# 2gunsu/monocon-pytorch

Measured on AMD Instinct MI355X. Metric: images/sec (384x1280) fwd+bwd, higher is better.
Workload: dtype f32 (f16x2); 1 GPU; train step B=32/GPU 3x384x1280 (configs[2] shape, fp32 values, mode f16x2); global_batch=32, parallelism=dp1, precision_mode=f16x2

## Files before the change

monocon-pytorch_amd/csrc/mc_internal.h:

```cpp
#pragma once
#include <hip/hip_runtime.h>

#include <cstdarg>
#include <cstdio>
#include <map>
#include <memory>
#include <string>
#include <tuple>
#include <unordered_map>
#include <vector>

#include "../../include/monocon_hip.h"
#include "conv_mfma.h"
#include "kernels.h"
#include "train.h"

using namespace mc;

struct TrainState;
struct CommState;

constexpr int MC_NUM_GRAD_BUCKETS = 4;
struct GradBucket {
    float *p = nullptr;
// ... 8 lines not shown
int mc_comm_join(mc_handle *h, hipStream_t main);

struct Bound {
    void *ptr;
    int64_t numel;
    int dtype;
};

struct Tensor {
    float *p = nullptr;
    int B = 0, H = 0, W = 0, C = 0;
    unsigned *amax = nullptr;
    const float *la = nullptr, *lb = nullptr;
    bool lrelu = true;
    size_t numel() const { return (size_t)B * H * W * C; }
};
inline Tensor operand_tensor(const float *p, int B, int H, int W, int C) {
    Tensor t;
    t.p = const_cast<float *>(p); t.B = B; t.H = H; t.W = W; t.C = C;
    return t;
}

struct ConvLayer {
    std::string conv, bn;
    int ks = 1, stride = 1, cin = 0, cout = 0, coutp = 0, cfg = 0;
    float bn_eps = 1e-5f;
    float *wpk = nullptr, *scale = nullptr, *shift = nullptr;
    void *wpk16 = nullptr;
    unsigned *w_amax = nullptr;
};

inline bool conv_fwd_args(ConvPlan &p, const ConvLayer &L, const std::vector<const Tensor *> &srcs, int prec) {
    ConvArgs &a = p.a;
    const Tensor &s0 = *srcs[0];
    a.nsrc = (int)srcs.size();
    a.Cin = 0;
    for (int i = 0; i < a.nsrc; ++i) {
        a.src[i] = ConvSrc{srcs[i]->p, srcs[i]->C, srcs[i]->la, srcs[i]->lb};
        a.Cin += srcs[i]->C;
    }
    a.B = s0.B; a.Hin = s0.H; a.Win = s0.W;
    a.Hout = conv_out_dim(s0.H, L.ks, L.stride); a.Wout = conv_out_dim(s0.W, L.ks, L.stride);
    a.Cout = L.cout; a.CoutP = L.coutp; a.wpk = L.wpk;
    a.wpk16 = L.wpk16; a.prec = L.wpk16 ? prec : 0;
    if (a.prec == 3) {
        for (int i = 0; i < a.nsrc; ++i) a.amax_in[i] = srcs[i]->amax;
        a.amax_w = L.w_amax;
    }
    p.ks = L.ks; p.stride = L.stride;
    conv_plan(p);
    return a.Cin == L.cin;
}
inline void wgrad_args(WgradPlan &p, const std::vector<const Tensor *> &srcs, const Tensor &dy, int dy_ld, int Cout, int ks,
                       int stride, int prec) {
    WgradArgs &a = p.a;
    const Tensor &s0 = *srcs[0];
    a.nsrc = (int)srcs.size();
    a.Cin = 0;
    for (int i = 0; i < a.nsrc; ++i) {
        a.src[i] = ConvSrc{srcs[i]->p, srcs[i]->C, srcs[i]->la, srcs[i]->lb};
        a.amax_x[i] = srcs[i]->amax;
        a.Cin += srcs[i]->C;
    }
    a.amax_dy = dy.amax;
    a.B = s0.B; a.Hin = s0.H; a.Win = s0.W; a.Hout = dy.H; a.Wout = dy.W; a.Cout = Cout;
    a.dy = dy.p; a.dy_ld = dy_ld;
    a.prec = prec; p.ks = ks; p.stride = stride;
    wgrad_plan(p);
}

struct DeconvLayer {
    std::string name;
    int C = 0;
    float *wpk = nullptr;
};

constexpr const char *HEAD_NAMES[NUM_HEADS] = {"heatmap_head", "wh_head", "offset_head", "center2kpt_offset_head",
                                               "kpt_heatmap_head", "kpt_heatmap_offset_head", "dim_head", "depth_head",
                                               "dir_feat"};
struct HeadOutLayer { std::string layer; int row0, rows; };
struct HeadKeys { std::string conv3, attn; std::vector<HeadOutLayer> out; };
inline HeadKeys mc_head_keys(int hd) {
    const std::string pre = std::string("head.") + HEAD_NAMES[hd];
    const int r0 = head_row_begin()[hd], nr = head_row_begin()[hd + 1] - r0;
    HeadKeys k{pre + ".0", pre + ".1", {{pre + ".3", r0, nr}}};
    if (hd == NUM_HEADS - 1) k.out = {{"head.dir_cls.0", r0, nr / 2}, {"head.dir_reg.0", r0 + nr / 2, nr / 2}};
    return k;
}

enum StepKind { STEP_CONV, STEP_POOL, STEP_DECONV };
struct NetStep {
    StepKind kind;
    std::string name, bn;
    std::vector<int> srcs;
    int res = -1;
    int out = -1;
    int ks = 1, stride = 1, cout = 0;
    bool relu = true;
    bool dead = false;
    bool elementwise_consumers = false;
    bool never_lazy = false;
};
struct NetGraph {
    std::vector<NetStep> steps;
    std::vector<int> node_c;
    int lv[6] = {};
    int n_backbone = 0;
    int feat = -1;
};

struct PlanMem {
    std::vector<void *> bufs;
    size_t bytes = 0;
    unsigned *amax_arena = nullptr;
    int amax_used = 0;
    void release() {
        for (void *q : bufs) (void)hipFree(q);
        bufs.clear();
    }
};
// ... 146 lines not shown
```

monocon-pytorch_amd/csrc/mc_train_api.hip:

```cpp
#include "mc_internal.h"

#include <algorithm>
#include <cmath>
#include <cstdlib>
#include <cstring>
#include <vector>

static int check_targets(mc_handle *h, const mc_targets *t, const char *who) {
    if (!t) return fail(h, "%s: targets is NULL", who);
    const void *p[] = {t->center_heatmap_target, t->wh_target, t->offset_target, t->dim_target, t->alpha_cls_target,
                       t->alpha_offset_target, t->depth_target, t->center2kpt_offset_target, t->kpt_heatmap_target,
                       t->kpt_heatmap_offset_target, t->indices, t->indices_kpt, t->mask_target,
                       t->mask_center2kpt_offset, t->mask_kpt_heatmap_offset};
    for (size_t i = 0; i < sizeof(p) / sizeof(p[0]); ++i)
        if (!p[i]) return fail(h, "%s: targets field %d is NULL", who, (int)i);
    return 0;
}

extern "C" {

int mc_make_targets(mc_handle *h, const mc_labels *lab, int B, int max_objs, int pad_h, int pad_w, int fh, int fw,
                    const mc_targets *t, void *stream) {
    if (!h) return -1;
    if (!lab || !lab->gt_bboxes || !lab->gt_labels || !lab->gt_bboxes_3d || !lab->depths || !lab->gt_kpts_2d ||
// ... 107 lines not shown
    HIPCHK(h, mc::launch_focal(preds[0], t->center_heatmap_target, (size_t)B * 3 * HW, h->loss_ws, scratch_losses + 0, aux + 0, st));
    HIPCHK(h, mc::launch_focal(preds[1], t->kpt_heatmap_target, (size_t)B * 9 * HW, h->loss_ws + npf, scratch_losses + 5, aux + 1, st));
    if (h->dp_arena && dpreds[2] == h->dp_arena) {
        HIPCHK(h, hipMemsetAsync(h->dp_arena, 0, h->dp_arena_bytes, st));
    } else {
        for (int i = 2; i < 10; ++i) HIPCHK(h, hipMemsetAsync(dpreds[i], 0, (size_t)B * mc::PRED_CH[i] * HW * 4, st));
    }
    HIPCHK(h, mc::launch_focal_grad(preds[0], t->center_heatmap_target, (size_t)B * 3 * HW, aux + 0, grad_losses, 0, dpreds[0], st, wrt_pred));
    HIPCHK(h, mc::launch_focal_grad(preds[1], t->kpt_heatmap_target, (size_t)B * 9 * HW, aux + 1, grad_losses, 5, dpreds[1], st, wrt_pred));
    mc::GatherLossArgs g{};
    fill_gather_args(g, preds, dpreds, t, B, max_objs, (int)HW, scratch_losses, aux + 2, grad_losses);
    g.wrt_pred = wrt_pred;
    g.partial = gather_ws(h);
    HIPCHK(h, mc::launch_gathered_losses(g, 1, st));
    return 0;
}

int mc_losses_backward(mc_handle *h, const float *const preds[MC_NUM_PREDS], const mc_targets *t, int B, int max_objs,
                       int fh, int fw, const float *grad_losses, float *const dpreds[MC_NUM_PREDS], void *stream) {
    return losses_backward_impl(h, preds, t, B, max_objs, fh, fw, grad_losses, dpreds, stream, 0);
}

int mc_losses_backward_pred(mc_handle *h, const float *const preds[MC_NUM_PREDS], const mc_targets *t, int B, int max_objs,
                            int fh, int fw, const float *grad_losses, float *const dpreds[MC_NUM_PREDS], void *stream) {
    return losses_backward_impl(h, preds, t, B, max_objs, fh, fw, grad_losses, dpreds, stream, 1);
}

int mc_op_conv_wgrad(mc_handle *h, const float *const src[], const int src_channels[], int nsrc, int B, int Hin, int Win,
                     const float *dy, int Cout, int ksize, int stride, float *dw_oihw, void *stream) {
    if (!h) return -1;
    if (!src || !src_channels || !dy || !dw_oihw || nsrc < 1 || nsrc > 4) return fail(h, "mc_op_conv_wgrad: bad argument");
    if (!((ksize == 3 && (stride == 1 || stride == 2)) || (ksize == 1 && stride == 1)))
        return fail(h, "mc_op_conv_wgrad: unsupported k=%d stride=%d", ksize, stride);
    if (Cout % 4) return fail(h, "mc_op_conv_wgrad: Cout must be a multiple of 4");
    HIPCHK(h, hipSetDevice(h->device));
    hipStream_t st = static_cast<hipStream_t>(stream);
    Tensor x[4];
    std::vector<const Tensor *> xs;
    for (int i = 0; i < nsrc; ++i) {
        if (!src[i] || src_channels[i] % 16) return fail(h, "mc_op_conv_wgrad: source %d needs C %% 16 == 0", i);
        x[i] = operand_tensor(src[i], B, Hin, Win, src_channels[i]);
        xs.push_back(&x[i]);
    }
    Tensor dyt = operand_tensor(dy, B, mc::conv_out_dim(Hin, ksize, stride), mc::conv_out_dim(Win, ksize, stride), Cout);
    ScratchBuf slots;
    if (h->prec == 3) {
        size_t n[4];
        for (int i = 0; i < nsrc; ++i) n[i] = x[i].numel();
        HIPCHK(h, op_amax_slots(slots, src, n, nsrc, dy, dyt.numel(), false, st));
        for (int i = 0; i < nsrc; ++i) x[i].amax = slots.as<unsigned>() + i * mc::AMAX_WORDS;
        dyt.amax = slots.as<unsigned>() + 4 * mc::AMAX_WORDS;
    }
    mc::WgradPlan p{};
    wgrad_args(p, xs, dyt, Cout, Cout, ksize, stride, h->prec);
    void *part = nullptr;
    HIPCHK(h, hipMalloc(&part, mc::wgrad_partial_floats(p) * sizeof(float)));
    p.a.partial = static_cast<float *>(part);
    hipError_t e = mc::launch_wgrad(p, dw_oihw, st);
    hipError_t e2 = hipStreamSynchronize(st);
    (void)hipFree(part);
    HIPCHK(h, e);
    HIPCHK(h, e2);
    return 0;
}

int mc_op_conv_dgrad(mc_handle *h, const float *dy, const float *weight_oihw, int B, int Hin, int Win, int CinTotal,
                     int c_off, int Cs, int Cout, int ksize, int stride, int accumulate, float *dx, void *stream) {
    if (!h) return -1;
    if (!dy || !weight_oihw || !dx) return fail(h, "mc_op_conv_dgrad: null argument");
    if (!((ksize == 3 && (stride == 1 || stride == 2)) || (ksize == 1 && stride == 1)))
        return fail(h, "mc_op_conv_dgrad: unsupported k=%d stride=%d", ksize, stride);
    if (Cout % 16 || Cs % 4 || c_off < 0 || c_off + Cs > CinTotal) return fail(h, "mc_op_conv_dgrad: bad channel arguments");
    if (stride == 2 && ((Hin | Win) & 1)) return fail(h, "mc_op_conv_dgrad: stride 2 needs even Hin, Win");
    HIPCHK(h, hipSetDevice(h->device));
    hipStream_t st = static_cast<hipStream_t>(stream);
    const int Ho = mc::conv_out_dim(Hin, ksize, stride), Wo = mc::conv_out_dim(Win, ksize, stride);
    const int nclass = stride == 2 ? 4 : 1;
    ScratchBuf slots;
    unsigned *dy_amax = nullptr, *w_amax = nullptr;
    if (h->prec == 3) {
        const size_t ndy = (size_t)B * Ho * Wo * Cout;
        HIPCHK(h, op_amax_slots(slots, &dy, &ndy, 1, weight_oihw, (size_t)Cout * CinTotal * ksize * ksize, true, st));
        dy_amax = slots.as<unsigned>();
        w_amax = dy_amax + 4 * mc::AMAX_WORDS;
    }
    ScratchBuf panel[4], panel16[4];
    mc::PackBatch pack;
    for (int c = 0; c < nclass; ++c) {
        const int cls = stride == 2 ? c : -1;
        const size_t pn = mc::dgrad_panel_elems(ksize, cls, Cout, Cs);
        HIPCHK(h, panel[c].alloc(pn * 4));
        HIPCHK(h, hipMemsetAsync(panel[c].p, 0, pn * 4, st));
        if (mc::panel_has_pieces(h->prec, Cout)) {
            const size_t bytes16 = pn * 2 * mc::split_pieces(h->prec);
            HIPCHK(h, panel16[c].alloc(bytes16));
            HIPCHK(h, hipMemsetAsync(panel16[c].p, 0, bytes16, st));
        }
        pack.add(mc::pack_job_dgrad(weight_oihw, Cout, CinTotal, ksize, c_off, Cs, Cout, cls, panel[c].as<float>(), panel16[c].p,
                                    h->prec, w_amax));
    }
    hipError_t e = pack.launch(st);
    for (int c = 0; c < nclass && e == hipSuccess; ++c) {
        mc::ConvPlan d;
        mc::dgrad_conv_args(d, pack.jobs[c], h->prec, dy, dy_amax, B, Ho, Wo, Cout, dx, Hin, Win, accumulate != 0);
        d.a.cfg = h->force_cfg;
        mc::conv_plan(d);
        e = mc::launch_conv(d, st);
// ... 165 lines not shown
```

monocon-pytorch_amd/csrc/mc_train_plan.hip:

```cpp
#include <atomic>
#include <deque>
#include <functional>

#include "mc_internal.h"

using namespace mc;

namespace {

using Fn = std::function<int(mc_handle *, hipStream_t)>;

struct PlanSwitches {
    long long lazy_z;
    long long lazy_min;
    long long lazy_feat;
    long long zbits;
    long long grad_pool;
    long long grad_pool_cool;
    long long head_dx_fuse;
    long long head_zskip;
    long long dgrad_s2_thin;
    long long stem_fuse;
    long long bm_epilogue;
    long long wres_bwd;
    long long dual_stream;
    int side_sync_lo = 0, side_sync_hi = 0;
    bool plan_debug = false;
};
const struct { const char *name; long long PlanSwitches::*field; long long def; } SWITCH_TABLE[] = {
    {"MONOCON_HIP_LAZY_Z", &PlanSwitches::lazy_z, 3},
    {"MONOCON_HIP_LAZY_MIN", &PlanSwitches::lazy_min, 900000},
    {"MONOCON_HIP_LAZY_FEAT", &PlanSwitches::lazy_feat, 0},
    {"MONOCON_HIP_ZBITS", &PlanSwitches::zbits, 1},
    {"MONOCON_HIP_GRAD_POOL", &PlanSwitches::grad_pool, 1},
    {"MONOCON_HIP_GRAD_POOL_COOL", &PlanSwitches::grad_pool_cool, 2},
    {"MONOCON_HIP_HEAD_DX_FUSE", &PlanSwitches::head_dx_fuse, 1},
    {"MONOCON_HIP_HEAD_ZSKIP", &PlanSwitches::head_zskip, 1},
    {"MONOCON_HIP_DGRAD_S2_THIN", &PlanSwitches::dgrad_s2_thin, 1},
    {"MONOCON_HIP_STEM_FUSE", &PlanSwitches::stem_fuse, 1},
    {"MONOCON_HIP_BM_EPILOGUE", &PlanSwitches::bm_epilogue, 1},
    {"MONOCON_HIP_WRES_BWD", &PlanSwitches::wres_bwd, 0},
    {"MONOCON_HIP_DUAL_STREAM", &PlanSwitches::dual_stream, 1},
};
PlanSwitches read_switches() {
    PlanSwitches sw{};
    std::string changed;
    for (const auto &d : SWITCH_TABLE) {
        const char *e = std::getenv(d.name);
        sw.*d.field = e ? std::atoll(e) : d.def;
        if (sw.*d.field != d.def) changed += std::string(" ") + d.name + "=" + std::to_string(sw.*d.field);
    }
    if (const char *e = std::getenv("MONOCON_HIP_SIDE_SYNC")) {
        if (std::sscanf(e, "%d:%d", &sw.side_sync_lo, &sw.side_sync_hi) != 2) sw.side_sync_lo = sw.side_sync_hi = 0;
        if (sw.side_sync_lo < sw.side_sync_hi) changed += std::string(" MONOCON_HIP_SIDE_SYNC=") + e;
    }
    sw.plan_debug = std::getenv("MONOCON_HIP_PLAN_DEBUG") != nullptr;
    if (sw.plan_debug && !changed.empty()) fprintf(stderr, "[plan] switches off their defaults:%s\n", changed.c_str());
    return sw;
}

struct PoolBwdArgs {
    const float *x, *dout, *la, *lb;
    float *dx, *stats;
    int B, H, W, C, acc;
};

struct LastWriter {
    enum Kind { NONE, DGRAD_CONV, POOL_BWD, DECONV_BWD } kind = NONE;
    union {
        ConvPlan *conv;
        PoolBwdArgs *pool;
        float **deconv_stats;
    };
    LastWriter() : conv(nullptr) {}
    LastWriter(ConvPlan *c) : kind(c ? DGRAD_CONV : NONE), conv(c) {}
    LastWriter(PoolBwdArgs *p) : kind(p ? POOL_BWD : NONE), pool(p) {}
    LastWriter(float **s) : kind(s ? DECONV_BWD : NONE), deconv_stats(s) {}
};

struct TNode {
    Tensor t;
    float *g = nullptr;
    bool ginit = false, needs_grad = true;
    LastWriter last;
};

enum RecKind { REC_STEM, REC_CONV, REC_POOL, REC_DECONV, REC_HEAD };
struct Rec {
    RecKind kind;
    ConvLayer *L = nullptr;
    DeconvLayer *D = nullptr;
    std::vector<int> srcs;
    int res = -1, z = -1, in = -1;
    bool relu = true, dead = false;
    Tensor y;
// ... 347 lines not shown
        float *dst = alloc(pn);
        void *dst16 = panel_has_pieces(h->prec, CoutPad) ? alloc((3 * pn + 1) / 2) : nullptr;
        ts->pack_batch.add(pack_job_dgrad(w, Cout, CinTotal, k, c_off, Cs, CoutPad, cls, dst, dst16, h->prec, w_slot(w)));
        return ts->pack_batch.jobs.back();
    }

    void emit_dgrad(const float *w_master, const Tensor &dy, int Cout_fwd, int CinTotal, int ks, int stride, int c_off, int srcnode,
                    int CoutPad) {
        TNode &sn = ts->nodes[srcnode];
        if (!sn.needs_grad) return;
        g_acquire(srcnode);
        auto dgrad_conv = [&](int cls, ConvPlan &d) {
            const PackJobDesc &p = pack_job(w_master, Cout_fwd, CinTotal, ks, c_off, sn.t.C, CoutPad, cls);
            dgrad_conv_args(d, p, h->prec, dy.p, dy.amax, dy.B, dy.H, dy.W, dy.C, sn.g, sn.t.H, sn.t.W, sn.ginit);
            d.a.cfg = ts->ok ? mc_choose_conv_cfg(h, d) : CFG_128x32;
        };
        if (stride == 2 && ks == 3) {
            if (2 * dy.H != sn.t.H || 2 * dy.W != sn.t.W) { ts->ok = false; h->err = "train plan: stride-2 dgrad shape mismatch"; }
            if (sw.dgrad_s2_thin && ts->ok && dgrad_s2_thin_ok(h->prec, ks, stride, dy.C, sn.t.C, CinTotal, c_off, dy.amax, w_slot(w_master), dy.H, dy.W)) {
                const float *dyp = dy.p;
                float *gp = sn.g;
                const int B = dy.B, Hd = dy.H, Wd = dy.W, Cd = dy.C, acc = sn.ginit ? 1 : 0;
                const unsigned *dmax = dy.amax, *wmax = w_slot(w_master);
                push_bwd([=](mc_handle *hh, hipStream_t st) {
                    HIPCHK(hh, launch_dgrad_s2_thin(dyp, B, Hd, Wd, Cd, w_master, CinTotal, c_off, gp, acc, dmax, wmax, st));
                    return 0;
                });
                wrote(srcnode);
                return;
            }
            for (int cls = 0; cls < 4; ++cls) {
                ConvPlan d;
                dgrad_conv(cls, d);
                conv_plan(d);
                push_bwd([=](mc_handle *hh, hipStream_t st) { HIPCHK(hh, launch_conv(d, st)); return 0; });
            }
            wrote(srcnode);
            return;
        }
        if (dy.H != sn.t.H || dy.W != sn.t.W) { ts->ok = false; h->err = "train plan: dgrad shape mismatch"; }
        ConvPlan d;
        dgrad_conv(-1, d);
        if (sw.wres_bwd < 2) d.a.cfg &= ~CFG_WRES;
        conv_plan(d);
        ts->dgrads.push_back(d);
        ConvPlan *dp = &ts->dgrads.back();
        push_bwd([=](mc_handle *hh, hipStream_t st) { HIPCHK(hh, launch_conv(*dp, st)); return 0; });
        wrote(srcnode, d.bm_ok ? dp : nullptr);
    }

    int emit_wgrad(const std::vector<int> &srcs, const Tensor &dy, int dy_ld, int Cout, int ks, int stride, float *dw) {
        WgradPlan p{};
        const std::vector<const Tensor *> xs = conv_sources(srcs);
        wgrad_args(p, xs, dy, dy_ld, Cout, ks, stride, h->prec);
        if (wgrad_any_lazy(p.a) && !wgrad_lazy_capable(p)) {
            for (int s_ : srcs) materialise(s_);
            wgrad_args(p, xs, dy, dy_ld, Cout, ks, stride, h->prec);
        }
        p.a.partial = alloc(wgrad_partial_floats(p));
        return push_bwd([=](mc_handle *hh, hipStream_t st) { HIPCHK(hh, launch_wgrad(p, dw, st)); return 0; }, ON_SIDE);
    }

    struct BnBwd { Tensor dy; float *coef; bool affine_skipped; };
    BnBwd bn_backward(const Rec &r, const std::string &bn, bool caller_forms_dy = false) {
        TNode &zn = ts->nodes[r.z];
        Tensor dy = r.y;
        dy.p = zn.g;
        dy.amax = slot();
        unsigned *dymax = dy.amax;
        const int B = r.y.B, C = r.y.C, rows = r.y.H * r.y.W;
        const float *yp = r.y.p, *gz = zn.g, *zp = zn.t.p, *gamma = P(bn + ".weight", C), *mean = r.mean, *rstd = r.rstd;
        float *dg = G(bn + ".weight", C), *db = G(bn + ".bias", C), *dyp = dy.p;
        float *coef = alloc((size_t)C * 4);
        const int relu = r.relu ? ((r.res < 0 && r.ca && r.cb) ? 2 : 1) : 0;
        const float *fa = r.ca, *fb = r.cb;
        float *gres = nullptr;
        int gmode = 0;
        if (r.res >= 0 && ts->nodes[r.res].needs_grad) {
            gres = g_acquire(r.res);
            gmode = ts->nodes[r.res].ginit ? 2 : 1;
            wrote(r.res);
        }
        const double n = (double)B * rows;
        auto step = [&](float *partial, int nbp, int cstride, bool reduce, bool affine) {
            double *fold = fold_scratch(nbp, C);
            const int arelu = reduce ? relu : 0;
            const float *aa = reduce ? fa : nullptr, *ab = reduce ? fb : nullptr;
            push_bwd([=](mc_handle *hh, hipStream_t st) {
                if (reduce) HIPCHK(hh, launch_chan_reduce(yp, gz, zp, nullptr, B, rows, C, 1, relu, partial, C, st, fa, fb));
                HIPCHK(hh, launch_bn_bwd_finalize(partial, nbp, cstride, n, C, gamma, mean, rstd, dg, db, coef, st, fold));
                if (affine)
                    HIPCHK(hh, launch_affine_bwd(gz, zp, yp, coef, B, (size_t)rows, C, 0, arelu, dyp, gres, gmode, st, aa, ab, nullptr,
                                                 nullptr, dymax));
                return 0;
            });
            return BnBwd{dy, coef, !affine};
        };
        const LastWriter last = zn.last;
        ConvPlan *lp = last.kind == LastWriter::DGRAD_CONV ? last.conv : nullptr;
        ConvArgs *lc = lp ? &lp->a : nullptr;
        if (sw.bm_epilogue == 0 || (sw.bm_epilogue > 1 && r.y.H * r.y.W > sw.bm_epilogue)) lc = nullptr;
        if (sw.plan_debug)
            fprintf(stderr, "[plan] bn_backward %-40s %4d ch %4dx%-4d relu %d res %d last-writer-conv %d\n", bn.c_str(), C, r.y.H,
                    r.y.W, relu, r.res >= 0, lc != nullptr);
        if (lc && lc->out == zn.g && lc->Cout == C && lc->out_ld == C && lc->Hout == r.y.H && lc->Wout == r.y.W && !lc->stats) {
            const int ppi = lp->stat_rows, nbp = B * ppi, cstride = lc->CoutP;
            float *partial = alloc((size_t)nbp * cstride * 2);
            lc->stats = partial;
            lc->bm_y = yp; lc->bm_z = zp; lc->bm_a = fa; lc->bm_b = fb; lc->bm_relu = relu;
            lc->bm_zbits = relu == 1 ? r.zbits : nullptr;
// ... 617 lines not shown
```

monocon-pytorch_amd/csrc/train.h:

```cpp
#pragma once
#include <hip/hip_runtime.h>
#include <stdint.h>
#include <cstdlib>
#include <vector>

#include "conv_mfma.h"

namespace mc {

struct TargetArgs {
    const float *gt_bboxes, *gt_labels, *gt_bboxes_3d, *depths, *gt_kpts_2d, *gt_kpts_valid, *mask;
    int B, max_objs, num_kpt, num_classes, fh, fw;
    float h_ratio, w_ratio;
    float *center_heatmap, *kpt_heatmap;
    float *wh, *offset, *dim, *alpha_cls, *alpha_offset, *depth, *c2k, *kho;
    long long *indices, *indices_kpt;
    uint8_t *mask_target;
    float *mask_c2k, *mask_kho;
};
hipError_t launch_make_targets(const TargetArgs &a, hipStream_t st);

hipError_t launch_focal(const float *p, const float *t, size_t n, float *partial, float *loss_out, float *aux,
                        hipStream_t st);
hipError_t launch_focal_grad(const float *p, const float *t, size_t n, const float *aux, const float *gscale, int gidx,
// ... 141 lines not shown
int affine_bwd_blocks(int B, size_t rows_per_img, int C);
size_t colsum_partial_floats(size_t rows, int ld);
hipError_t launch_colsum(const float *x, size_t rows, int C, int ld, float *partial, float *out, hipStream_t st);
hipError_t launch_colsum_final(const float *partial, int nb, int C, float *out, hipStream_t st);
hipError_t launch_maxpool2_bwd(const float *x, const float *dout, int B, int H, int W, int C, float *dx, int accumulate,
                               hipStream_t st, const float *la = nullptr, const float *lb = nullptr,
                               float *stats_partial = nullptr);
int maxpool2_bwd_blocks(int B, int H, int W, int C);
size_t deconv4_bwd_w_partial_floats(int B, int H, int C);
hipError_t launch_deconv4_bwd_w(const float *in, const float *dout, int B, int H, int W, int C, float *partial, float *dw,
                                hipStream_t st, const float *la, const float *lb,
                                const float *wpk, float *din,
                                float *stats = nullptr);

hipError_t launch_dpred_pack(const float *const dpred[10], int ld, int B, int HW, float *out, hipStream_t st,
                             unsigned *nz = nullptr);
hipError_t launch_dpred_pack_user(const float *const dpred[10], const float *const pred[10], const float *const grad[10], int ld,
                                  int B, int HW, float *out, hipStream_t st, unsigned *nz = nullptr);
struct AttnTrainArgs {
    const float *stats;
    int chunks, stat_ld, B, HW;
    double *stats64;
    float *rm[9], *rv[9];
    long long *nbt[9];
    const float *att_w[9], *att_g[9], *att_b[9];
    float *att_rm[9], *att_rv[9];
    long long *att_nbt[9];
    const float *weight_[9], *bias_[9];
    float *sv_inst;
    float *mu_r;
    float *bn10;
    float *that, *yatt;
    float *gamma_p;
    float *scale, *shift;
};
struct AttnGradPtrs { float *d_weight_[9], *d_bias_[9], *d_att_w[9], *d_att_g[9], *d_att_b[9]; };
hipError_t launch_attn_train_fwd(const AttnTrainArgs &a, hipStream_t st);
hipError_t launch_attn_train_bwd(const AttnTrainArgs &a, const float *partial, int rb_per_img, const AttnGradPtrs &gp,
                                 float *coef, hipStream_t st);
hipError_t launch_head_bwd(const float *draw, int ld, const float *z, const float *x, const float *w1, int B, int HW,
                           int blocks, float *d, float *dw_partial, float *red_partial, hipStream_t st,
                           const float *scale = nullptr, const float *shift = nullptr, const unsigned *nz = nullptr);
hipError_t launch_head_dx(const float *draw, int ld, const float *x, const float *w1, const float *coef, int B, int HW, int blocks,
                          float *dx, float *csum, float *csum_out, unsigned *amax, hipStream_t st, const float *scale,
                          const float *shift, const unsigned *nz = nullptr);
hipError_t launch_splitk_reduce(const float *partial, int ksplit, int T, int Cout, int Cin, float *dw, hipStream_t st);
int stem_wgrad_blocks(int B, int H, int W);
hipError_t launch_stem_wgrad(const float *img, const float *dy, int B, int H, int W, float *partial, float *dw,
                             hipStream_t st, const unsigned *img_amax = nullptr, const unsigned *dy_amax = nullptr,
                             const float *y = nullptr, const float *coef = nullptr, const unsigned *y_amax = nullptr);
hipError_t launch_stem_dgrad(const float *dy, const float *w_oihw, int B, int H, int W, float *dx, hipStream_t st,
                             const float *y = nullptr, const float *coef = nullptr);

enum WgKernel { WG_FP32, WG_SPLIT, WG_PIPE, WG_SMALL, WG_THIN16 };
struct WgradArgs {
    ConvSrc src[4];
    int nsrc;
    int B, Hin, Win, Hout, Wout, Cin, Cout;
    const float *dy;
    int dy_ld;
    float *partial;
    int ksplit, n_tiles, c_tiles, ppr, ppi, groups_per_img;
    int kernel;
    int prec;
    int pb;
    int pipe;
    const unsigned *amax_x[4], *amax_dy;
};
static_assert(sizeof(WgradArgs) == 264, "WgradArgs is the kernels' parameter block: keep its layout");
struct WgradPlan {
    WgradArgs a;
    int ks, stride;
    int WN, WC;
    bool lazy_ok;
    bool ok;
    size_t partial_floats;
};
inline void wgrad_set_patches(WgradArgs &a, int pb) {
    a.ppr = (a.Wout + 7) / 8;
    a.ppi = a.ppr * ((a.Hout + 3) / 4);
    a.groups_per_img = (a.ppi + pb - 1) / pb;
}
inline bool wgrad_any_lazy(const WgradArgs &a) { return any_lazy_src(a.src, a.nsrc); }
template <int WN_, int WC_>
struct WgTile { static constexpr int WN = WN_, WC = WC_; };
template <typename F>
inline hipError_t with_wgrad_tile(int WN, int WC, F &&f) {
    if (WN == 2 && WC == 2) return f(WgTile<2, 2>{});
    if (WN == 4) return f(WgTile<4, 1>{});
    if (WN == 2) return f(WgTile<2, 1>{});
    return f(WgTile<1, 1>{});
}
inline size_t wgrad_lds_request(size_t need) {
#ifdef MC_DEBUG_HOOKS
    static const size_t pad = [] { const char *e = std::getenv("MONOCON_HIP_WGRAD_LDS_KB"); return e ? (size_t)std::atoi(e) * 1024 : (size_t)0; }();
    return pad > need ? pad : need;
#else
    return need;
#endif
}
void wgrad_plan(WgradPlan &p);
hipError_t launch_wgrad(const WgradPlan &p, float *dw_oihw, hipStream_t st);
inline size_t wgrad_partial_floats(const WgradPlan &p) { return p.partial_floats; }
inline bool wgrad_lazy_capable(const WgradPlan &p) { return p.lazy_ok; }
bool wgrad_is_small(const WgradArgs &a, int ks, int stride);
bool wgrad_thin_ok(const WgradArgs &a, int ks, int stride);
int wgrad_pipe_tile(const WgradArgs &a, int ks, int stride);
void wgrad_shape(const WgradArgs &a, int *WN, int *WC);
bool wgrad_sources_ok(const WgradArgs &a);
bool wgrad_bf16_ok(const WgradArgs &a, int ks, int stride);
hipError_t launch_wgrad_fp32(const WgradPlan &p, hipStream_t st);
hipError_t launch_wgrad_small(const WgradPlan &p, hipStream_t st);
hipError_t launch_wgrad_bf16(const WgradPlan &p, hipStream_t st);
hipError_t launch_wgrad_pipe(const WgradPlan &p, hipStream_t st);
hipError_t launch_wgrad_thin(const WgradPlan &p, hipStream_t st);

}
```

monocon-pytorch_amd/csrc/wgrad_plan.hip:

```cpp
#include <algorithm>
#include <cstdlib>
#include "conv_mfma.h"
#include "train.h"

namespace mc {

static int env_int(const char *name, int unset) { const char *e = std::getenv(name); return e ? std::atoi(e) : unset; }

void wgrad_plan(WgradPlan &p) {
    WgradArgs &a = p.a;
    const int ks = p.ks, stride = p.stride;
    a.pipe = p.WN = p.WC = 0; p.ok = true;
    if (wgrad_is_small(a, ks, stride)) {
        a.kernel = wgrad_thin_ok(a, ks, stride) ? WG_THIN16 : WG_SMALL;
        p.lazy_ok = a.prec == 3 && (a.kernel == WG_THIN16 || (stride == 2 && a.Cout == 32));
        const int rows = a.B * a.Hout;
        a.ksplit = std::min(rows / 4 > 0 ? rows / 4 : 1, 1024);
        a.n_tiles = a.c_tiles = 1; a.ppr = a.ppi = a.groups_per_img = 0;
    } else {
        int budget, WK = 1;
        if (const int tile = wgrad_pipe_tile(a, ks, stride)) {
            a.kernel = WG_PIPE; a.pipe = tile; a.pb = 1;
            p.WN = tile == 1 ? 4 : 2; p.WC = tile == 2 ? 4 : 2; WK = tile == 3 ? 2 : 1;
            p.lazy_ok = tile == 4;
            budget = env_int("MONOCON_HIP_WGRAD_PIPE_BLOCKS", 256);
        } else {
            wgrad_shape(a, &p.WN, &p.WC);
            const bool b16 = a.prec >= 1 && wgrad_bf16_ok(a, ks, stride), src_ok = wgrad_sources_ok(a);
            a.kernel = b16 ? WG_SPLIT : WG_FP32;
            a.pb = (b16 && a.prec >= 2) ? 1 : 2;
            p.lazy_ok = a.prec == 3 && b16 && src_ok;
            p.ok = src_ok && (b16 || (ks == 3 && (stride == 1 || stride == 2)) || (ks == 1 && stride == 1));
            budget = env_int("MONOCON_HIP_WGRAD_BLOCKS", 512) * 4 / (p.WN * p.WC);
        }
        a.n_tiles = (a.Cout + 32 * p.WN - 1) / (32 * p.WN);
        a.c_tiles = (a.Cin + 32 * p.WC - 1) / (32 * p.WC);
        wgrad_set_patches(a, a.pb);
        const long long G = (long long)a.B * a.groups_per_img;
        a.ksplit = (int)std::min<long long>(std::max(budget / (a.n_tiles * a.c_tiles), 1), G) * WK;
    }
    if (wgrad_any_lazy(a) && !p.lazy_ok) p.ok = false;
    p.partial_floats = (size_t)a.ksplit * ks * ks * a.Cout * a.Cin;
}

hipError_t launch_wgrad(const WgradPlan &p, float *dw_oihw, hipStream_t st) {
    const WgradArgs &a = p.a;
    if (!p.ok) return hipErrorInvalidValue;
    prof_last = {2, 2.0 * a.B * a.Hout * a.Wout * (double)a.Cout * a.Cin * p.ks * p.ks,
                 4.0 * ((double)a.B * a.Hin * a.Win * a.Cin + (double)a.B * a.Hout * a.Wout * a.Cout + (double)p.ks * p.ks * a.Cin * a.Cout)};
    hipError_t e = hipErrorInvalidValue;
    switch (a.kernel) {
    case WG_FP32: e = launch_wgrad_fp32(p, st); break;
    case WG_SPLIT: e = launch_wgrad_bf16(p, st); break;
    case WG_PIPE: e = launch_wgrad_pipe(p, st); break;
    case WG_SMALL: e = launch_wgrad_small(p, st); break;
    case WG_THIN16: e = launch_wgrad_thin(p, st); break;
    }
    if (e != hipSuccess) return e;
    return launch_splitk_reduce(a.partial, a.ksplit, p.ks * p.ks, a.Cout, a.Cin, dw_oihw, st);
}

}
```

scratch/wgrad_plan_dump.hip:

```cpp
#include <cstdio>
#include <cstdlib>
#include <cstring>
#include <string>
#include <vector>
#include "train.h"

using namespace mc;

struct Case { std::string name; int B, H, W; std::vector<int> cins; int Cout, ks, stride, dy_ld = 0; bool amax = true; };

static unsigned g_slot[4];
static bool g_probe = false, g_kernels = false;

static void fill(WgradArgs &a, const Case &c, int prec, int lazy) {
    a.nsrc = (int)c.cins.size();
    a.Cin = 0;
    const float *f = reinterpret_cast<const float *>(g_slot);
    for (int i = 0; i < a.nsrc; ++i) {
        const bool lz = lazy == 1 || (lazy == 2 && i == 0);
        a.src[i] = ConvSrc{f, c.cins[i], lz ? f : nullptr, lz ? f : nullptr};
        a.amax_x[i] = (prec == 3 && c.amax) ? g_slot : nullptr;
        a.Cin += c.cins[i];
    }
    a.amax_dy = (prec == 3 && c.amax) ? g_slot : nullptr;
    a.B = c.B; a.Hin = c.H; a.Win = c.W;
    a.Hout = conv_out_dim(c.H, c.ks, c.stride); a.Wout = conv_out_dim(c.W, c.ks, c.stride);
    a.Cout = c.Cout; a.dy = f; a.dy_ld = c.dy_ld ? c.dy_ld : c.Cout;
    a.prec = prec;
}

static void dump(const Case &c, int prec, int lazy) {
    size_t partial;
    bool lazy_ok;
    int small, pipe, bf16;
    hipError_t e = hipSuccess;
    char extra[64] = "";
#ifdef WGRAD_DUMP_OLD_API
    WgradArgs a{};
    fill(a, c, prec, lazy);
    wgrad_plan(a, c.ks, c.stride);
    partial = wgrad_partial_floats(a, c.ks);
    lazy_ok = wgrad_lazy_capable(a, c.ks, c.stride);
    small = a.small; pipe = a.pipe;
    bf16 = !a.small && !a.pipe && a.prec >= 1 && wgrad_bf16_ok(a, c.ks, c.stride);
    if (g_probe) e = launch_wgrad(a, c.ks, c.stride, nullptr, 0);
#else
    WgradPlan p{};
    fill(p.a, c, prec, lazy);
    p.ks = c.ks; p.stride = c.stride;
    wgrad_plan(p);
    const WgradArgs &a = p.a;
    partial = wgrad_partial_floats(p);
    lazy_ok = wgrad_lazy_capable(p);
    small = a.kernel == WG_SMALL || a.kernel == WG_THIN16; pipe = a.pipe; bf16 = a.kernel == WG_SPLIT;
    if (g_probe) e = launch_wgrad(p, nullptr, 0);
    static const char *const names[] = {"fp32", "split", "pipe", "small", "thin16"};
    if (g_kernels) std::snprintf(extra, sizeof extra, " kernel=%s waves=%dx%d", names[a.kernel], p.WN, p.WC);
#endif
    std::printf("%s prec=%d lazy=%d ksplit=%d n_tiles=%d c_tiles=%d pb=%d ppr=%d ppi=%d groups_per_img=%d partial=%zu lazy_ok=%d "
                "small=%d pipe=%d bf16=%d launch=%s%s\n",
                c.name.c_str(), prec, lazy, a.ksplit, a.n_tiles, a.c_tiles, a.pb, a.ppr, a.ppi, a.groups_per_img, partial, (int)lazy_ok,
                small, pipe, bf16, !g_probe ? "-" : (e == hipErrorInvalidValue ? "invalid" : "ok"), extra);
}

static void train_plan_cases(std::vector<Case> &out, int B, int H, int W) {
    char tag[32];
    std::snprintf(tag, sizeof tag, "plan_b%d_%dx%d", B, H, W);
    auto add = [&](const char *what, int level, std::vector<int> cins, int Cout, int ks, int stride, int dy_ld = 0) {
        out.push_back({std::string(tag) + "_" + what, B, H >> level, W >> level, std::move(cins), Cout, ks, stride, dy_ld});
    };
    add("level0", 0, {16}, 16, 3, 1);
    add("level1", 0, {16}, 32, 3, 2);
    const int ch[6] = {16, 32, 64, 128, 256, 512};
    for (int lv = 2; lv <= 5; ++lv) {
        const int ci = ch[lv - 1], co = ch[lv];
        const std::string l = "level" + std::to_string(lv);
        add((l + "_down").c_str(), lv - 1, {ci}, co, 3, 2);
        add((l + "_block").c_str(), lv, {co}, co, 3, 1);
        add((l + "_project").c_str(), lv, {ci}, co, 1, 1);
        add((l + "_root").c_str(), lv, lv == 5 ? std::vector<int>{co, co, ci} : std::vector<int>{co, co}, co, 1, 1);
        if (lv == 3 || lv == 4) add((l + "_root4").c_str(), lv, {co, co, ci, co}, co, 1, 1);
    }
    for (int lv = 5; lv >= 3; --lv) {
        const int co = ch[lv - 1];
        add(("ida_proj_" + std::to_string(ch[lv]) + "_" + std::to_string(co)).c_str(), lv, {ch[lv]}, co, 3, 1);
        add(("ida_node_" + std::to_string(co)).c_str(), lv - 1, {co, co}, co, 3, 1);
    }
    add("heads_64_576", 2, {64}, 576, 3, 1, 576);
}

static void test_cases(std::vector<Case> &out) {
    out.insert(out.end(), {
        {"wg_s1_64_64", 2, 16, 24, {64}, 64, 3, 1}, {"wg_s1_128_128", 2, 12, 40, {128}, 128, 3, 1},
        {"wg_s1_cat_64_64_to64", 2, 8, 16, {64, 64}, 64, 3, 1}, {"wg_s1_16_16", 1, 20, 24, {16}, 16, 3, 1},
        {"wg_s1_odd", 1, 6, 10, {32}, 64, 3, 1}, {"wg_s2_32_64", 2, 16, 32, {32}, 64, 3, 2}, {"wg_s2_16_32", 1, 24, 16, {16}, 32, 3, 2},
        {"wg_s2_256_512", 1, 8, 8, {256}, 512, 3, 2}, {"wg_k1_root4", 1, 12, 16, {128, 128, 64, 128}, 128, 1, 1},
        {"wg_k1_32_64", 2, 8, 8, {32}, 64, 1, 1}, {"wg_head_64_576", 1, 8, 16, {64}, 576, 3, 1},
        {"wg_s2_128_256_24x48", 2, 24, 48, {128}, 256, 3, 2}, {"wg_s1_256_256_12x24", 2, 12, 24, {256}, 256, 3, 1},
        {"wg_s2_64_128_48x96", 2, 48, 96, {64}, 128, 3, 2},
        {"b16wg_64_64", 2, 16, 24, {64}, 64, 3, 1}, {"b16wg_128_128", 2, 12, 40, {128}, 128, 3, 1},
        {"b16wg_cat_64_64", 2, 8, 16, {64, 64}, 64, 3, 1}, {"b16wg_odd_edges", 1, 6, 10, {32}, 64, 3, 1},
        {"b16wg_head_64_576", 1, 8, 16, {64}, 576, 3, 1}, {"b16wg_k1_root4", 1, 12, 16, {128, 128, 64, 128}, 128, 1, 1},
        {"b16wg_k1_32_64", 2, 8, 8, {32}, 64, 1, 1}, {"b16wg_256_256_12x24", 2, 12, 24, {256}, 256, 3, 1},
        {"b16wg_128_64", 1, 8, 16, {128}, 64, 3, 1}, {"b16wg_odd_64_128", 1, 6, 10, {64}, 128, 3, 1},
        {"b16wg_cat_64_64_128", 1, 10, 20, {64, 64}, 128, 3, 1},
        {"s2_32_64", 2, 16, 32, {32}, 64, 3, 2}, {"s2_64_128", 1, 24, 48, {64}, 128, 3, 2}, {"s2_128_256", 2, 8, 16, {128}, 256, 3, 2},
        {"s2_ragged_patches", 1, 10, 24, {64}, 64, 3, 2}, {"s2_256_512", 1, 12, 40, {256}, 512, 3, 2},
        {"s2_two_sources", 1, 16, 16, {32, 32}, 64, 3, 2}});
}
// ... 56 lines not shown
```

Baseline: 679.9 images/sec.

## Add streaming MFMA wgrad kernel for 1x1 stride-1 convolutions

Adds a dedicated weight-gradient kernel for 1x1 stride-1 convolutions in the fp16-split precision mode. It streams pixel chunks through a four-deep register prefetch and a double-buffered LDS tile, splitting each value into hi/lo f16 parts for three MFMAs. The planner now routes eligible layers to it by default, with its own split-k budget. The aim is to replace the generic pipe/split wgrad path, which pays im2col-style overhead on pointwise convs. This adds a new code path with its own accuracy and occupancy trade-offs.

```diff
diff --git a/monocon-pytorch_amd/csrc/mc_internal.h b/monocon-pytorch_amd/csrc/mc_internal.h
--- a/monocon-pytorch_amd/csrc/mc_internal.h
+++ b/monocon-pytorch_amd/csrc/mc_internal.h
@@ -84,7 +84,7 @@
     return a.Cin == L.cin;
 }
 inline void wgrad_args(WgradPlan &p, const std::vector<const Tensor *> &srcs, const Tensor &dy, int dy_ld, int Cout, int ks,
-                       int stride, int prec) {
+                       int stride, int prec, int stream_1x1) {
     WgradArgs &a = p.a;
     const Tensor &s0 = *srcs[0];
     a.nsrc = (int)srcs.size();
@@ -97,7 +97,7 @@
     a.amax_dy = dy.amax;
     a.B = s0.B; a.Hin = s0.H; a.Win = s0.W; a.Hout = dy.H; a.Wout = dy.W; a.Cout = Cout;
     a.dy = dy.p; a.dy_ld = dy_ld;
-    a.prec = prec; p.ks = ks; p.stride = stride;
+    a.prec = prec; p.ks = ks; p.stride = stride; p.stream_1x1 = stream_1x1;
     wgrad_plan(p);
 }
 
diff --git a/monocon-pytorch_amd/csrc/mc_train_api.hip b/monocon-pytorch_amd/csrc/mc_train_api.hip
--- a/monocon-pytorch_amd/csrc/mc_train_api.hip
+++ b/monocon-pytorch_amd/csrc/mc_train_api.hip
@@ -183,7 +183,7 @@
         dyt.amax = slots.as<unsigned>() + 4 * mc::AMAX_WORDS;
     }
     mc::WgradPlan p{};
-    wgrad_args(p, xs, dyt, Cout, Cout, ksize, stride, h->prec);
+    wgrad_args(p, xs, dyt, Cout, Cout, ksize, stride, h->prec, mc::wgrad_1x1_stream_env());
     void *part = nullptr;
     HIPCHK(h, hipMalloc(&part, mc::wgrad_partial_floats(p) * sizeof(float)));
     p.a.partial = static_cast<float *>(part);
diff --git a/monocon-pytorch_amd/csrc/mc_train_plan.hip b/monocon-pytorch_amd/csrc/mc_train_plan.hip
--- a/monocon-pytorch_amd/csrc/mc_train_plan.hip
+++ b/monocon-pytorch_amd/csrc/mc_train_plan.hip
@@ -24,6 +24,7 @@
     long long bm_epilogue;
     long long wres_bwd;
     long long dual_stream;
+    long long wgrad_1x1_stream;
     int side_sync_lo = 0, side_sync_hi = 0;
     bool plan_debug = false;
 };
@@ -41,6 +42,7 @@
     {"MONOCON_HIP_BM_EPILOGUE", &PlanSwitches::bm_epilogue, 1},
     {"MONOCON_HIP_WRES_BWD", &PlanSwitches::wres_bwd, 0},
     {"MONOCON_HIP_DUAL_STREAM", &PlanSwitches::dual_stream, 1},
+    {"MONOCON_HIP_WGRAD_1X1_STREAM", &PlanSwitches::wgrad_1x1_stream, 1},
 };
 PlanSwitches read_switches() {
     PlanSwitches sw{};
@@ -494,10 +496,10 @@
     int emit_wgrad(const std::vector<int> &srcs, const Tensor &dy, int dy_ld, int Cout, int ks, int stride, float *dw) {
         WgradPlan p{};
         const std::vector<const Tensor *> xs = conv_sources(srcs);
-        wgrad_args(p, xs, dy, dy_ld, Cout, ks, stride, h->prec);
+        wgrad_args(p, xs, dy, dy_ld, Cout, ks, stride, h->prec, (int)sw.wgrad_1x1_stream);
         if (wgrad_any_lazy(p.a) && !wgrad_lazy_capable(p)) {
             for (int s_ : srcs) materialise(s_);
-            wgrad_args(p, xs, dy, dy_ld, Cout, ks, stride, h->prec);
+            wgrad_args(p, xs, dy, dy_ld, Cout, ks, stride, h->prec, (int)sw.wgrad_1x1_stream);
         }
         p.a.partial = alloc(wgrad_partial_floats(p));
         return push_bwd([=](mc_handle *hh, hipStream_t st) { HIPCHK(hh, launch_wgrad(p, dw, st)); return 0; }, ON_SIDE);
diff --git a/monocon-pytorch_amd/csrc/train.h b/monocon-pytorch_amd/csrc/train.h
--- a/monocon-pytorch_amd/csrc/train.h
+++ b/monocon-pytorch_amd/csrc/train.h
@@ -217,7 +217,7 @@
 hipError_t launch_stem_dgrad(const float *dy, const float *w_oihw, int B, int H, int W, float *dx, hipStream_t st,
                              const float *y = nullptr, const float *coef = nullptr);
 
-enum WgKernel { WG_FP32, WG_SPLIT, WG_PIPE, WG_SMALL, WG_THIN16 };
+enum WgKernel { WG_FP32, WG_SPLIT, WG_PIPE, WG_SMALL, WG_THIN16, WG_STREAM1X1 };
 struct WgradArgs {
     ConvSrc src[4];
     int nsrc;
@@ -236,6 +236,7 @@
 struct WgradPlan {
     WgradArgs a;
     int ks, stride;
+    int stream_1x1;
     int WN, WC;
     bool lazy_ok;
     bool ok;
@@ -266,8 +267,11 @@
 }
 void wgrad_plan(WgradPlan &p);
 hipError_t launch_wgrad(const WgradPlan &p, float *dw_oihw, hipStream_t st);
+int wgrad_1x1_stream_env();
 inline size_t wgrad_partial_floats(const WgradPlan &p) { return p.partial_floats; }
 inline bool wgrad_lazy_capable(const WgradPlan &p) { return p.lazy_ok; }
+bool wgrad_1x1_ok(const WgradArgs &a, int ks, int stride);
+int wgrad_1x1_wc(const WgradArgs &a, int *c_tiles);
 bool wgrad_is_small(const WgradArgs &a, int ks, int stride);
 bool wgrad_thin_ok(const WgradArgs &a, int ks, int stride);
 int wgrad_pipe_tile(const WgradArgs &a, int ks, int stride);
@@ -279,5 +283,6 @@
 hipError_t launch_wgrad_bf16(const WgradPlan &p, hipStream_t st);
 hipError_t launch_wgrad_pipe(const WgradPlan &p, hipStream_t st);
 hipError_t launch_wgrad_thin(const WgradPlan &p, hipStream_t st);
-
-}
+hipError_t launch_wgrad_1x1(const WgradPlan &p, hipStream_t st);
+
+}
diff --git a/monocon-pytorch_amd/csrc/wgrad_1x1.hip b/monocon-pytorch_amd/csrc/wgrad_1x1.hip
--- /dev/null
+++ b/monocon-pytorch_amd/csrc/wgrad_1x1.hip
@@ -0,0 +1,242 @@
+#include "conv_mfma.h"
+#include "train.h"
+
+namespace mc {
+
+typedef _Float16 s1_h16x8 __attribute__((ext_vector_type(8)));
+template <int V> struct S1Int { static constexpr int value = V; };
+
+template <int WN, int WC>
+struct Wg1x1Cfg {
+    static constexpr int NB = 32 * WN, CB = 32 * WC, NT = 64 * WN * WC;
+    static constexpr int CHUNK = 32, DEPTH = 4;
+    static constexpr int ROW = 4 * 16 + 48;
+    static constexpr int X_PLANE = CB * ROW, D_PLANE = NB * ROW;
+    static constexpr int BUF = 2 * (X_PLANE + D_PLANE);
+    static constexpr size_t LDS_BYTES = 2 * BUF;
+    static_assert(2 * LDS_BYTES <= 160 * 1024, "two workgroups per CU");
+};
+
+__device__ __forceinline__ int s1_skew(int channel) { return ((channel >> 4) & 3) * 16; }
+__device__ __forceinline__ int s1_lane_chan(int li) { return ((li & 15) >= 4 && (li & 15) < 12) ? (li ^ 16) : li; }
+
+__device__ __forceinline__ void s1_split_pair(float x0, float x1, float s, unsigned &hi, unsigned &lo) {
+    unsigned h, l;
+    asm("v_fma_mixlo_f16 %0, %1, %2, 0" : "=v"(h) : "v"(x0), "v"(s));
+    asm("v_fma_mixhi_f16 %0, %1, %2, 0" : "+v"(h) : "v"(x1), "v"(s));
+    asm("v_fma_mixlo_f16 %0, %1, %2, -%3 op_sel_hi:[0,0,1]" : "=v"(l) : "v"(x0), "v"(s), "v"(h));
+    asm("v_fma_mixhi_f16 %0, %1, %2, -%3 op_sel:[0,0,1] op_sel_hi:[0,0,1]" : "+v"(l) : "v"(x1), "v"(s), "v"(h));
+    hi = h;
+    lo = l;
+}
+
+__device__ __forceinline__ void s1_barrier() { asm volatile("s_waitcnt lgkmcnt(0)\n\ts_barrier" ::: "memory"); }
+
+__host__ __device__ __forceinline__ int s1_src_tiles(int C, int CB) { return (C + CB - 1) / CB; }
+
+template <int WN, int WC, bool LZ>
+__global__ __launch_bounds__(64 * WN * WC, 2) void wgrad_1x1_kernel(const WgradArgs a) {
+    using Cfg = Wg1x1Cfg<WN, WC>;
+    constexpr int NB = Cfg::NB, CB = Cfg::CB, NT = Cfg::NT, CHUNK = Cfg::CHUNK, DEPTH = Cfg::DEPTH, ROW = Cfg::ROW;
+    constexpr int XPL = Cfg::X_PLANE, DPL = Cfg::D_PLANE, BUF = Cfg::BUF;
+    static_assert(DEPTH == 4, "the loop below is unrolled over four register sets and two tile buffers");
+    extern __shared__ __attribute__((aligned(16))) unsigned char lds_raw[];
+
+    const int tid = threadIdx.x, lane = tid & 63;
+    const int wave = __builtin_amdgcn_readfirstlane(tid >> 6);
+    const int wn = wave / WC, wc = wave % WC;
+    const int g = lane >> 5, li = lane & 31;
+    const int bid = xcd_order(blockIdx.x, gridDim.x);
+    const int ct = __builtin_amdgcn_readfirstlane(bid % a.c_tiles);
+    const int nt = __builtin_amdgcn_readfirstlane((bid / a.c_tiles) % a.n_tiles);
+    const int ks = __builtin_amdgcn_readfirstlane(bid / (a.c_tiles * a.n_tiles));
+    const int n0 = nt * NB;
+
+    int si = 0, cbase = 0, tl = ct;
+    while (si + 1 < a.nsrc && tl >= s1_src_tiles(a.src[si].C, CB)) { tl -= s1_src_tiles(a.src[si].C, CB); cbase += a.src[si].C; ++si; }
+    const int Cs = a.src[si].C, cs0 = tl * CB;
+
+    const long long P = (long long)a.B * a.Hout * a.Wout;
+    const int nch = (int)((P + CHUNK - 1) / CHUNK);
+    const int ch_begin = __builtin_amdgcn_readfirstlane((int)((long long)nch * ks / a.ksplit));
+    const int ch_end = __builtin_amdgcn_readfirstlane((int)((long long)nch * (ks + 1) / a.ksplit));
+    const long long p_begin = (long long)ch_begin * CHUNK;
+    const long long p_end = (long long)ch_end * CHUNK < P ? (long long)ch_end * CHUNK : P;
+    const unsigned npix = p_end > p_begin ? (unsigned)(p_end - p_begin) : 0u;
+    const __amdgpu_buffer_rsrc_t r_x = make_rsrc(a.src[si].p + p_begin * Cs, npix * (unsigned)Cs * 4u);
+    const __amdgpu_buffer_rsrc_t r_d = make_rsrc(a.dy + p_begin * a.dy_ld, npix * (unsigned)a.dy_ld * 4u);
+
+    const int ex = f16_scale_exp(amax_read(a.amax_x[si])), ed = f16_scale_exp(amax_read(a.amax_dy));
+    const float x_scale = exp2i(ex), d_scale = exp2i(ed), omul = exp2i(-ex) * exp2i(-ed);
+
+    constexpr int XC4 = CB / 4, NC4 = NB / 4, NIX = 16 * XC4 / NT, NID = 16 * NC4 / NT;
+    static_assert(NIX * NT == 16 * XC4 && NID * NT == 16 * NC4 && NT % XC4 == 0 && NT % NC4 == 0, "whole items, static channel quad per thread");
+    const int xq = tid % XC4, dq = tid % NC4;
+    const bool xc_ok = cs0 + xq * 4 < Cs;
+    const bool dn_ok = n0 + dq * 4 + 3 < a.dy_ld;
+    const int x_px = Cs * 4, d_px = a.dy_ld * 4;
+    const int x_step = xc_ok ? CHUNK * x_px : 0, d_step = dn_ok ? CHUNK * d_px : 0;
+    int x_off[NIX], x_dst[NIX], d_off[NID], d_dst[NID];
+#pragma unroll
+    for (int i = 0; i < NIX; ++i) {
+        const int item = (tid + NT * i) / XC4, row8 = item >> 2, pp = item & 3;
+        x_off[i] = xc_ok ? ((row8 * 8 + pp * 2) * Cs + cs0 + xq * 4) * 4 : BUF_OOB;
+        x_dst[i] = (xq * 4) * ROW + s1_skew(xq * 4) + row8 * 16 + pp * 4;
+    }
+#pragma unroll
+    for (int i = 0; i < NID; ++i) {
+        const int item = (tid + NT * i) / NC4, row8 = item >> 2, pp = item & 3;
+        d_off[i] = dn_ok ? ((row8 * 8 + pp * 2) * a.dy_ld + n0 + dq * 4) * 4 : BUF_OOB;
+        d_dst[i] = 2 * XPL + (dq * 4) * ROW + s1_skew(dq * 4) + row8 * 16 + pp * 4;
+    }
+
+    const bool lz = LZ && a.src[si].la != nullptr;
+    [[maybe_unused]] f32x4 lzA = {0.f, 0.f, 0.f, 0.f}, lzB = lzA;
+    if constexpr (LZ) {
+        if (lz && xc_ok) {
+            lzA = *reinterpret_cast<const f32x4 *>(a.src[si].la + cs0 + xq * 4);
+            lzB = *reinterpret_cast<const f32x4 *>(a.src[si].lb + cs0 + xq * 4);
+#pragma unroll
+            for (int j = 0; j < 4; ++j) { lzA[j] *= x_scale; lzB[j] *= x_scale; }
+        }
+    }
+
+    f32x4 xv[DEPTH][NIX][2], dv[DEPTH][NID][2];
+    auto fetch = [&](auto slot_c) {
+        constexpr int slot = decltype(slot_c)::value;
+#pragma unroll
+        for (int i = 0; i < NIX; ++i) {
+            xv[slot][i][0] = buf_load4(r_x, x_off[i], 0);
+            xv[slot][i][1] = buf_load4(r_x, x_off[i] + x_px, 0);
+            x_off[i] += x_step;
+        }
+#pragma unroll
+        for (int i = 0; i < NID; ++i) {
+            dv[slot][i][0] = buf_load4(r_d, d_off[i], 0);
+            dv[slot][i][1] = buf_load4(r_d, d_off[i] + d_px, 0);
+            d_off[i] += d_step;
+        }
+    };
+    auto put = [&](unsigned char *dst, int plane, const f32x4 v0, const f32x4 v1, float scale) {
+#pragma unroll
+        for (int j = 0; j < 4; ++j) {
+            unsigned hi, lo;
+            s1_split_pair(v0[j], v1[j], scale, hi, lo);
+            *reinterpret_cast<unsigned *>(dst + j * ROW) = hi;
+            *reinterpret_cast<unsigned *>(dst + plane + j * ROW) = lo;
+        }
+    };
+    auto stage = [&](unsigned char *buf, auto slot_c) {
+        constexpr int slot = decltype(slot_c)::value;
+#pragma unroll
+        for (int i = 0; i < NIX; ++i) {
+            if constexpr (LZ) {
+                if (lz) {
+                    f32x4 t0, t1;
+#pragma unroll
+                    for (int j = 0; j < 4; ++j) {
+                        t0[j] = lazy_act(xv[slot][i][0][j], lzA[j], lzB[j], __builtin_inff());
+                        t1[j] = lazy_act(xv[slot][i][1][j], lzA[j], lzB[j], __builtin_inff());
+                    }
+                    put(buf + x_dst[i], XPL, t0, t1, 1.f);
+                    continue;
+                }
+            }
+            put(buf + x_dst[i], XPL, xv[slot][i][0], xv[slot][i][1], x_scale);
+        }
+#pragma unroll
+        for (int i = 0; i < NID; ++i) put(buf + d_dst[i], DPL, dv[slot][i][0], dv[slot][i][1], d_scale);
+    };
+
+    f32x16 acc_main, acc_minor;
+#pragma unroll
+    for (int r = 0; r < 16; ++r) acc_main[r] = acc_minor[r] = 0.f;
+    const int lc = s1_lane_chan(li);
+    const int a_off = 2 * XPL + (wn * 32 + lc) * ROW + s1_skew(wn * 32 + lc) + g * 16;
+    const int b_off = (wc * 32 + lc) * ROW + s1_skew(wc * 32 + lc) + g * 16;
+    auto mfmas = [&](const unsigned char *buf) {
+#pragma unroll
+        for (int q = 0; q < 2; ++q) {
+            s1_h16x8 av[2], bv[2];
+#pragma unroll
+            for (int z = 0; z < 2; ++z) {
+                av[z] = *reinterpret_cast<const s1_h16x8 *>(buf + a_off + z * DPL + q * 32);
+                bv[z] = *reinterpret_cast<const s1_h16x8 *>(buf + b_off + z * XPL + q * 32);
+            }
+            acc_minor = __builtin_amdgcn_mfma_f32_32x32x16_f16(av[1], bv[0], acc_minor, 0, 0, 0);
+            acc_minor = __builtin_amdgcn_mfma_f32_32x32x16_f16(av[0], bv[1], acc_minor, 0, 0, 0);
+            acc_main = __builtin_amdgcn_mfma_f32_32x32x16_f16(av[0], bv[0], acc_main, 0, 0, 0);
+        }
+    };
+    auto iteration = [&](auto cur_c, auto sn) {
+        unsigned char *cur = lds_raw + decltype(cur_c)::value * BUF, *nxt = lds_raw + (1 - decltype(cur_c)::value) * BUF;
+        mfmas(cur);
+        stage(nxt, sn);
+        __builtin_amdgcn_sched_barrier(0);
+        fetch(sn);
+        s1_barrier();
+    };
+
+    const int n = ch_end - ch_begin;
+    if (n > 0) {
+        fetch(S1Int<0>{});
+        __builtin_amdgcn_sched_barrier(0);
+        fetch(S1Int<1>{});
+        __builtin_amdgcn_sched_barrier(0);
+        fetch(S1Int<2>{});
+        __builtin_amdgcn_sched_barrier(0);
+        fetch(S1Int<3>{});
+        __builtin_amdgcn_sched_barrier(0);
+        stage(lds_raw, S1Int<0>{});
+        __builtin_amdgcn_sched_barrier(0);
+        fetch(S1Int<0>{});
+        s1_barrier();
+    }
+    for (int i = 0; i < n; i += DEPTH) {
+        iteration(S1Int<0>{}, S1Int<1>{});
+        iteration(S1Int<1>{}, S1Int<2>{});
+        iteration(S1Int<0>{}, S1Int<3>{});
+        iteration(S1Int<1>{}, S1Int<0>{});
+    }
+
+    const int cl = cs0 + wc * 32 + lc;
+    if (cl < Cs) {
+#pragma unroll
+        for (int r = 0; r < 16; ++r) {
+            const int nn = n0 + wn * 32 + s1_lane_chan((r & 3) + 8 * (r >> 2) + 4 * g);
+            if (nn < a.Cout) a.partial[((size_t)ks * a.Cout + nn) * a.Cin + cbase + cl] = (acc_main[r] + acc_minor[r]) * omul;
+        }
+    }
+}
+
+bool wgrad_1x1_ok(const WgradArgs &a, int ks, int stride) {
+    if (a.prec != 3 || ks != 1 || stride != 1 || a.Hout != a.Hin || a.Wout != a.Win) return false;
+    if (a.nsrc < 1 || a.nsrc > 4 || a.dy_ld % 4 || a.dy_ld < a.Cout || !a.amax_dy) return false;
+    const long long P = (long long)a.B * a.Hout * a.Wout, lim = 1ll << 31;
+    if ((P + 512) * a.dy_ld * 4 >= lim) return false;
+    for (int i = 0; i < a.nsrc; ++i)
+        if (!a.amax_x[i] || a.src[i].C % 4 || (P + 512) * a.src[i].C * 4 >= lim) return false;
+    return true;
+}
+int wgrad_1x1_wc(const WgradArgs &a, int *c_tiles) {
+    int WC = 2;
+    for (int i = 0; i < a.nsrc; ++i)
+        if (a.src[i].C % 64) WC = 1;
+    *c_tiles = 0;
+    for (int i = 0; i < a.nsrc; ++i) *c_tiles += s1_src_tiles(a.src[i].C, 32 * WC);
+    return WC;
+}
+
+template <int WN, int WC>
+static hipError_t launch_s1(const WgradArgs &a, hipStream_t st) {
+    using Cfg = Wg1x1Cfg<WN, WC>;
+    const dim3 grid(a.ksplit * a.n_tiles * a.c_tiles);
+    if (wgrad_any_lazy(a)) return launch_dyn_lds<wgrad_1x1_kernel<WN, WC, true>>(wgrad_lds_request(Cfg::LDS_BYTES), grid, dim3(Cfg::NT), st, a);
+    return launch_dyn_lds<wgrad_1x1_kernel<WN, WC, false>>(wgrad_lds_request(Cfg::LDS_BYTES), grid, dim3(Cfg::NT), st, a);
+}
+hipError_t launch_wgrad_1x1(const WgradPlan &p, hipStream_t st) {
+    if (p.WN != 2) return hipErrorInvalidValue;
+    return p.WC == 2 ? launch_s1<2, 2>(p.a, st) : (p.WC == 1 ? launch_s1<2, 1>(p.a, st) : hipErrorInvalidValue);
+}
+
+}
diff --git a/monocon-pytorch_amd/csrc/wgrad_plan.hip b/monocon-pytorch_amd/csrc/wgrad_plan.hip
--- a/monocon-pytorch_amd/csrc/wgrad_plan.hip
+++ b/monocon-pytorch_amd/csrc/wgrad_plan.hip
@@ -6,12 +6,22 @@
 namespace mc {
 
 static int env_int(const char *name, int unset) { const char *e = std::getenv(name); return e ? std::atoi(e) : unset; }
+int wgrad_1x1_stream_env() { return env_int("MONOCON_HIP_WGRAD_1X1_STREAM", 1); }
 
 void wgrad_plan(WgradPlan &p) {
     WgradArgs &a = p.a;
     const int ks = p.ks, stride = p.stride;
     a.pipe = p.WN = p.WC = 0; p.ok = true;
-    if (wgrad_is_small(a, ks, stride)) {
+    if (p.stream_1x1 && wgrad_1x1_ok(a, ks, stride)) {
+        a.kernel = WG_STREAM1X1; a.pb = 1;
+        p.WN = 2; p.WC = wgrad_1x1_wc(a, &a.c_tiles);
+        p.lazy_ok = true;
+        a.n_tiles = (a.Cout + 63) / 64;
+        wgrad_set_patches(a, a.pb);
+        const long long chunks = ((long long)a.B * a.Hout * a.Wout + 31) / 32;
+        const int budget = env_int("MONOCON_HIP_WGRAD_BLOCKS", 512) * (p.WC == 1 ? 3 : 2) / 2;
+        a.ksplit = (int)std::min<long long>(std::max(budget / (a.n_tiles * a.c_tiles), 1), chunks);
+    } else if (wgrad_is_small(a, ks, stride)) {
         a.kernel = wgrad_thin_ok(a, ks, stride) ? WG_THIN16 : WG_SMALL;
         p.lazy_ok = a.prec == 3 && (a.kernel == WG_THIN16 || (stride == 2 && a.Cout == 32));
         const int rows = a.B * a.Hout;
@@ -55,6 +65,7 @@
     case WG_PIPE: e = launch_wgrad_pipe(p, st); break;
     case WG_SMALL: e = launch_wgrad_small(p, st); break;
     case WG_THIN16: e = launch_wgrad_thin(p, st); break;
+    case WG_STREAM1X1: e = launch_wgrad_1x1(p, st); break;
     }
     if (e != hipSuccess) return e;
     return launch_splitk_reduce(a.partial, a.ksplit, p.ks * p.ks, a.Cout, a.Cin, dw_oihw, st);
diff --git a/scratch/wgrad_plan_dump.hip b/scratch/wgrad_plan_dump.hip
--- a/scratch/wgrad_plan_dump.hip
+++ b/scratch/wgrad_plan_dump.hip
@@ -47,14 +47,14 @@
 #else
     WgradPlan p{};
     fill(p.a, c, prec, lazy);
-    p.ks = c.ks; p.stride = c.stride;
+    p.ks = c.ks; p.stride = c.stride; p.stream_1x1 = wgrad_1x1_stream_env();
     wgrad_plan(p);
     const WgradArgs &a = p.a;
     partial = wgrad_partial_floats(p);
     lazy_ok = wgrad_lazy_capable(p);
     small = a.kernel == WG_SMALL || a.kernel == WG_THIN16; pipe = a.pipe; bf16 = a.kernel == WG_SPLIT;
     if (g_probe) e = launch_wgrad(p, nullptr, 0);
-    static const char *const names[] = {"fp32", "split", "pipe", "small", "thin16"};
+    static const char *const names[] = {"fp32", "split", "pipe", "small", "thin16", "stream1x1"};
     if (g_kernels) std::snprintf(extra, sizeof extra, " kernel=%s waves=%dx%d", names[a.kernel], p.WN, p.WC);
 #endif
     std::printf("%s prec=%d lazy=%d ksplit=%d n_tiles=%d c_tiles=%d pb=%d ppr=%d ppi=%d groups_per_img=%d partial=%zu lazy_ok=%d "
```

Result: no change. 681.3 images/sec, median of 4 (+0.2%).
